# PlatonB/ld-tools

Measured on AMD Instinct MI355X. Metric: SNP-pairs/sec (r2+D'), higher is better.
Workload: dtype fp4 (E2M1 0/1 operands, exact f32 accumulation)

## Files before the change

### ld_tools_amd/csrc/ldx_mfma.hip

```cpp
#include <stdlib.h>
#include <string.h>

#include <atomic>
#include <type_traits>

#include "ldx_common.h"
#include "ldx_tile.h"

namespace ldx {

typedef int v4i __attribute__((ext_vector_type(4)));
typedef int v16i __attribute__((ext_vector_type(16)));
typedef unsigned v4u __attribute__((ext_vector_type(4)));
typedef unsigned v2u __attribute__((ext_vector_type(2)));
typedef float v4f __attribute__((ext_vector_type(4)));
typedef int v8i __attribute__((ext_vector_type(8)));
typedef float v16f __attribute__((ext_vector_type(16)));

__device__ __forceinline__ void gload16_s(v4u &dst, uint32_t voff, const void *sbase)
{
    const void *t;
    asm volatile("s_mov_b64 %1, %3\n\tglobal_load_dwordx4 %0, %2, %1" : "=v"(dst), "=&s"(t) : "v"(voff), "s"(sbase));
}
__device__ __forceinline__ void gload16x2_s(v4u &dst0, v4u &dst1, uint32_t voff, const void *sbase)
// ... 290 lines not shown
                const uint32_t x = (my_xcd + k) & 7u;
                const uint32_t lo = aa.pass_base[(uint32_t)((uint64_t)n_slabs * x / 8u)], hi = aa.pass_base[(uint32_t)((uint64_t)n_slabs * (x + 1u) / 8u)];
                if (lo == hi) continue;
                const uint32_t got = atomicAdd(&sched[2u + 32u * x], 1u);
                if (got < hi - lo) return aa.order ? aa.order[lo + got] : lo + got;
            }
            return 0xFFFFFFFFu;
        } else {
            if (!sched) return static_next += gridDim.x;
            return gridDim.x + atomicAdd(&sched[0], 1u);
        }
    };
    uint32_t *ktok = nullptr;
    if (!kArea && sched && (ablate_arg & 4096)) {
        const uint32_t hw = __builtin_amdgcn_s_getreg(63492), xcc = __builtin_amdgcn_s_getreg(63508);
        ktok = sched + 2u + ((((xcc & 7u) * 8u + ((hw >> 13) & 7u)) * 2u + ((hw >> 12) & 1u)) * 16u + ((hw >> 8) & 15u));
    }
    uint32_t parity = 0;
    if (tid == 0) tickets[0] = kArea ? draw() : blockIdx.x;

    uint64_t hit_slot = 0, hit_slot_end = 0;
    uint32_t t_prev = 0xFFFFFFFFu;
    for (;;) {
        block_sync();
        const uint32_t ticket = tickets[parity];
        parity ^= 1u;
        if (kArea ? ticket == 0xFFFFFFFFu : ticket >= n_tickets) {
            if (tid == 0 && sched && atomicAdd(&sched[1], 1u) == gridDim.x - 1u) {
                store_agent(&sched[1], 0u);
                if (kArea)
                    for (uint32_t x = 0; x < 8u; ++x) store_agent(&sched[2u + 32u * x], 0u);
                asm volatile("s_waitcnt vmcnt(0)" ::: "memory");
                store_agent(&sched[0], 0u);
            }
            break;
        }
        const bool short_pass = !kArea && ticket >= n_norm;
        const uint32_t hsel = short_pass ? (ticket - n_norm) & 1u : 0u;
        const uint32_t seq = short_pass ? n_norm + ((ticket - n_norm) >> 1) : ticket;
        uint32_t p = p_begin + seq;
        auto pbase = [&](uint32_t tile) { return kArea ? aa.pass_base[tile] : mfma_pass_base(tile, n_slabs); };
        auto tile_of_pass = [&](uint32_t pp) {
            uint32_t lo = 0, hi = n_slabs;
            while (hi - lo > 1) {
                const uint32_t mid = (lo + hi) / 2;
                if (pbase(mid) <= pp) lo = mid; else hi = mid;
            }
            return lo;
        };
        uint32_t t;
        if (kArea && (ticket & kAreaDecoded)) {
            t = (ticket >> 12) & 0xFFFu;
            p = pbase(t) + (ticket & 0xFFFu);
        } else
#ifndef LDX_AB_FORWARD_TILES
        if constexpr (!kArea) {
            const uint32_t mirrored = p_end - 1u - seq;
            t = tile_of_pass(mirrored);
            const uint32_t lo_t = pbase(t) > p_begin ? pbase(t) : p_begin;
            const uint32_t hi_t = (t + 1u < n_slabs && pbase(t + 1u) < p_end) ? pbase(t + 1u) : p_end;
            p = lo_t + (hi_t - 1u - mirrored);
        } else
#endif
        {
            t = tile_of_pass(p);
        }
        const bool new_tile = t != t_prev;
        t_prev = t;
        const uint64_t tb = base64(t), te = base64(t + 1u);
        const uint64_t area_first = kArea ? tb + (aa.g_begin[t] - 2u * t) : 0u;
        const uint64_t pass = (kArea ? area_first : tb) + (uint64_t)(p - pbase(t)) * kMfmaWaves;
        const uint64_t seg_begin = kArea ? area_first : (v_begin > tb ? v_begin : tb);
        const uint64_t seg_end = kArea ? tb + (aa.g_end[t] > 2u * t ? aa.g_end[t] - 2u * t : 0u) : (v_end < te ? v_end : te);
        const uint32_t b_off = kFp4 ? ((tid >> 7) * kSlab + (tid & 127u)) * 16u : (tid >> 1) * kBRow + (tid & 1u) * 64u;
        const uint32_t nblocks = kFp4 ? nchunks / 2u : nchunks;

        auto pass_body = [&](auto mm_c) {
            constexpr int MM = decltype(mm_c)::value;
            const uint64_t vv = pass + wave;
            const bool active = vv >= seg_begin && vv < seg_end;
            const uint32_t g64 = (uint32_t)((vv < te ? vv : pass) - tb) + 2u * t;
            const uint32_t roff = MM == 1 ? 32u * hsel : 0u;
            const uint32_t row0 = g64 * kRows64 + roff;
            const uint4 *ai = alt + ((size_t)(row0 / kSlab) * nchunks) * kSlab + (row0 % kSlab) + l32 + (kFp4 ? half * kSlab : 0u);
            constexpr uint32_t kAStride = kFp4 ? 2u * kSlab : kSlab;

            typedef std::conditional_t<kFp4, v16f, v16i> acc_t;
            typedef std::conditional_t<kFp4, float, int> accel_t;
            auto count_of = [](accel_t x) { if constexpr (kFp4) return (uint32_t)x; else return (uint32_t)x >> 3; };
            acc_t acc[MM][4];
#pragma unroll
            for (int m = 0; m < MM; ++m)
#pragma unroll
                for (int tt = 0; tt < 4; ++tt)
#pragma unroll
                    for (int e = 0; e < 16; ++e) acc[m][tt][e] = 0;

            auto read_bf = [&](v4i (&bf)[4], const unsigned char *buf, int w) {
#pragma unroll
                for (int tt = 0; tt < 4; ++tt)
#ifdef LDX_AB_NOBREAD
                    bf[tt] = v4i{(int)(uintptr_t)buf + w + tt, 1, 1, 1};
#else
                    bf[tt] = kFp4 ? *reinterpret_cast<const v4i *>(buf + (((uint32_t)w * 2u + half) * kSlab + 32u * tt + l32) * 16u)
                                  : *reinterpret_cast<const v4i *>(buf + (32u * tt + l32) * kBRow + w * 32u + half * 16u);
#endif
            };
            auto mma8 = [&](const v4i (&af)[MM], const v4i (&bf)[4]) {
#pragma unroll
                for (int m = 0; m < MM; ++m)
#pragma unroll
                    for (int tt = 0; tt < 4; ++tt)
#ifdef LDX_AB_NOMFMA
                        asm volatile("" : "+v"(acc[m][tt]) : "v"(af[m]), "v"(bf[tt]));
#else
                    {
                        if constexpr (kFp4) {
                            const v8i a8v = {af[m].x, af[m].y, af[m].z, af[m].w, 0, 0, 0, 0};
                            const v8i b8v = {bf[tt].x, bf[tt].y, bf[tt].z, bf[tt].w, 0, 0, 0, 0};
                            acc[m][tt] = __builtin_amdgcn_mfma_scale_f32_32x32x64_f8f6f4(a8v, b8v, acc[m][tt], 4, 4, 0, 0, 0, 0);
                        } else {
                            acc[m][tt] = __builtin_amdgcn_mfma_i32_32x32x32_i8(af[m], bf[tt], acc[m][tt], 0, 0, 0);
                        }
                    }
#endif
            };
            auto interleave = [&]() {
                __builtin_amdgcn_sched_group_barrier(0x100, 4, 0);
#pragma unroll
                for (int k = 0; k < 4 * MM; ++k) {
                    __builtin_amdgcn_sched_group_barrier(0x008, 1, 0);
                    __builtin_amdgcn_sched_group_barrier(0x002, LDX_VALU_PER_MFMA, 0);
                }
            };
            auto lds_barrier = [&]() {
                __builtin_amdgcn_sched_barrier(0);
#ifndef LDX_AB_NOBARRIER
                __builtin_amdgcn_s_waitcnt(0xC07F);
                __builtin_amdgcn_s_barrier();
#endif
                __builtin_amdgcn_sched_barrier(0);
            };

            LDX_STAMP(0);
            v4u ar[3][MM];
            auto touch_ring = [&](int k) {
                if constexpr (MM == 2) asm volatile("" : "+v"(ar[k][0]), "+v"(ar[k][1]));
                else asm volatile("" : "+v"(ar[k][0]));
            };
            typedef std::conditional_t<kFp4, v4u, v2u> bring_t;
            bring_t br[3];
            auto clampc = [&](uint32_t c) { return c < nblocks ? c : nblocks - 1u; };
            constexpr uint32_t kBlockBytes = kAStride * 16u;
            const uint32_t b_voff = kFp4 ? (uint32_t)((((size_t)t * nchunks + (tid >> 7)) * kSlab + (tid & 127u)) * 16u)
                                         : (uint32_t)(((size_t)t * nchunks * kSlab) * 16u + tid * 8u);
            const uint32_t a_voff = (uint32_t)((size_t)(ai - alt) * 16u);
            auto block_base = [&](uint32_t blk) { return reinterpret_cast<const unsigned char *>(alt) + (size_t)blk * kBlockBytes; };
            auto load_b = [&](bring_t &dst, uint32_t blk) {
                if constexpr (kFp4) gload16_s(dst, b_voff, block_base(blk));
                else gload8_s(dst, b_voff, block_base(blk));
            };
            auto load_a = [&](v4u (&dst)[MM], uint32_t blk) {
                if constexpr (MM == 2) gload16x2_s(dst[0], dst[1], a_voff, block_base(blk));
                else gload16_s(dst[0], a_voff, block_base(blk));
            };
            auto bquarter = [&](unsigned char *buf, const bring_t &bits, int q) {
// ... 97 lines not shown
            block_sync();
            LDX_STAMP(1);
            if (ablate & 32) __builtin_amdgcn_s_setprio(2);
#if defined(LDX_AB_BANDPRIO)
            if (kArea) { if (LDX_AB_BANDPRIO == 1 ? (blockIdx.x >= gridDim.x / 2u) : (blockIdx.x & 1u)) __builtin_amdgcn_s_setprio(1); else __builtin_amdgcn_s_setprio(0); }
#endif
            v4i af0[MM], bf0[4], af1[MM], bf1[4];
            read_bf(bf0, bexp, 0);
#pragma unroll
            for (int m = 0; m < MM; ++m) af0[m] = expand_a(ar[0][m].x);

            const uint32_t nch_run = (ablate & 2) ? 1u : nblocks;
#ifdef LDX_CHUNK_STAMPS
            unsigned long long cst[6] = {0, 0, 0, 0, 0, 0};
#endif
#define LDX_CHUNK(CUR, NXT, FAR, cc)                                                                               \
            {                                                                                                      \
                const uint32_t c_ = (cc);                                                                          \
                const unsigned char *rd = bexp + (c_ & 1u) * kBBuf;                                                \
                unsigned char *wr = bexp + ((c_ + 1u) & 1u) * kBBuf;                                               \
                const uint32_t c3 = clampc(c_ + 2u);                                                               \
                LDX_CSTAMP(0)                                                                                      \
                 \
                       \
                load_b(br[FAR], c3);                                                                               \
                load_a(ar[FAR], c3);                                                                               \
                asm volatile("s_waitcnt vmcnt(%0)" : : "n"(MM == 2 ? 5 : 3));    \
                asm volatile("" : "+v"(br[NXT]));                                                                  \
                      \
                read_bf(bf1, rd, 1);                                                                               \
                _Pragma("unroll") for (int m = 0; m < MM; ++m) af1[m] = expand_a(ar[CUR][m].y);               \
                bquarter(wr, br[NXT], 1);                                                                          \
                mma8(af0, bf0);                                                                                    \
                interleave();                                                                                      \
                __builtin_amdgcn_sched_barrier(0);                                                                 \
                LDX_CSTAMP(1)                                                                                      \
                                             \
                read_bf(bf0, rd, 2);                                                                               \
                _Pragma("unroll") for (int m = 0; m < MM; ++m) af0[m] = expand_a(ar[CUR][m].z);               \
                bquarter(wr, br[NXT], 2);                                                                          \
                mma8(af1, bf1);                                                                                    \
                interleave();                                                                                      \
                __builtin_amdgcn_sched_barrier(0);                                                                 \
                LDX_CSTAMP(2)                                                                                      \
                                             \
                read_bf(bf1, rd, 3);                                                                               \
                _Pragma("unroll") for (int m = 0; m < MM; ++m) af1[m] = expand_a(ar[CUR][m].w);               \
                bquarter(wr, br[NXT], 3);                                                                          \
                mma8(af0, bf0);                                                                                    \
                interleave();                                                                                      \
                __builtin_amdgcn_sched_barrier(0);                                                                 \
                LDX_CSTAMP(3)                                                                                      \
                lds_barrier();                        \
                LDX_CSTAMP(4)                                                                                      \
                   \
                 \
                           \
                asm volatile("s_waitcnt vmcnt(%0)" : : "n"(MM));                                                   \
                touch_ring(NXT);                                                                                   \
                asm volatile("" : "+v"(br[FAR]));                                                                  \
                read_bf(bf0, wr, 0);                                                                               \
                _Pragma("unroll") for (int m = 0; m < MM; ++m) af0[m] = expand_a(ar[NXT][m].x);               \
                bquarter(bexp + (c_ & 1u) * kBBuf, br[FAR], 0);                                                    \
                mma8(af1, bf1);                                                                                    \
                interleave();                                                                                      \
                __builtin_amdgcn_sched_barrier(0);                                                                 \
                LDX_CSTAMP(5)                                                                                      \
            }
#define LDX_CHUNK_IDLE(NXT, FAR, cc)                                                                               \
            {                                                                                                      \
                const uint32_t c_ = (cc);                                                                          \
                unsigned char *wr = bexp + ((c_ + 1u) & 1u) * kBBuf;                                               \
                load_b(br[FAR], clampc(c_ + 2u));                                                                  \
                asm volatile("s_waitcnt vmcnt(1)");                                 \
                asm volatile("" : "+v"(br[NXT]));                                                                  \
                bquarter(wr, br[NXT], 1);                                                                          \
                bquarter(wr, br[NXT], 2);                                                                          \
                bquarter(wr, br[NXT], 3);                                                                          \
                lds_barrier();                                                                                     \
                asm volatile("s_waitcnt vmcnt(0)");                                                                \
                asm volatile("" : "+v"(br[FAR]));                                                                  \
                bquarter(bexp + (c_ & 1u) * kBBuf, br[FAR], 0);                                                    \
            }
            if (__builtin_expect(!active, 0)) {
                for (uint32_t c = 0; c < nch_run; c += 3) {
                    LDX_CHUNK_IDLE(1, 2, c)
                    if (c + 1 < nch_run) LDX_CHUNK_IDLE(2, 0, c + 1)
                    if (c + 2 < nch_run) LDX_CHUNK_IDLE(0, 1, c + 2)
                }
            } else {
#ifdef LDX_AB_PEEL
            if constexpr (!kArea) {
                LDX_CHUNK(0, 1, 2, 0u)
                for (uint32_t c = 1; c < nch_run; c += 3) {
                    LDX_CHUNK(1, 2, 0, c)
                    if (c + 1 < nch_run) LDX_CHUNK(2, 0, 1, c + 1)
                    if (c + 2 < nch_run) LDX_CHUNK(0, 1, 2, c + 2)
                }
            } else
#endif
            {
                for (uint32_t c = 0; c < nch_run; c += 3) {
                    LDX_CHUNK(0, 1, 2, c)
                    if (c + 1 < nch_run) LDX_CHUNK(1, 2, 0, c + 1)
                    if (c + 2 < nch_run) LDX_CHUNK(2, 0, 1, c + 2)
                }
            }
            }
#undef LDX_CHUNK
#undef LDX_CHUNK_IDLE
            asm volatile("s_waitcnt vmcnt(0)");
            touch_ring(0);
            touch_ring(1);
            touch_ring(2);
            asm volatile("" : "+v"(br[0]), "+v"(br[1]), "+v"(br[2]));

#ifdef LDX_CHUNK_STAMPS
            asm volatile("s_waitcnt lgkmcnt(0)");
            if (my_stamps && lane == 0 && npass == 1)
                for (int k = 0; k < 6; ++k) my_stamps[6 + 4 * (kStampPasses - 2) + k] = cst[k];
#endif
            LDX_STAMP(2);
            uint32_t next_ticket = 0;
            if (tid == 0) {
                if (ktok) atomicExch(ktok, 0u);
                next_ticket = draw();
            }
            if (ablate & 32) __builtin_amdgcn_s_setprio(0);
            else if (!(ablate & 16)) __builtin_amdgcn_s_setprio(3);
            if constexpr (kScore) {
                block_sync();
            } else if (!active) {
                if (tid == 0) tickets[parity] = next_ticket;
                return;
            }
            typedef double d2 __attribute__((ext_vector_type(2)));
            double fa2[4], fr2[4];
            double sfa = 0.0, sfr = 0.0, sq = 0.0;
#pragma unroll
            for (int tt = 0; tt < 4; ++tt) {
                if (kRaw) {
                    fa2[tt] = fa[t * kSlab + 32u * tt + l32];
                    fr2[tt] = fr[t * kSlab + 32u * tt + l32];
                }
            }
            if (kRaw) {
                const uint32_t il = row0 + (MM == 1 ? l32 : lane);
                sfa = fa[il];
                sfr = fr[il];
                sq = q[il];
            }
            auto epilogue = [&](auto clean_c) {
#pragma unroll 1
            for (int e = 0; e < 16; ++e) {
                constexpr bool kClean = decltype(clean_c)::value;
                uint32_t ri[MM], cnt[MM][4];
                uint64_t us[MM];
                bool in_range[MM], valid[MM][4], slow[MM][4];
                Cell res[MM][4];
                ldx_ld64 rw[MM][4];
                bool any_slow = false;
#pragma unroll
                for (int m = 0; m < MM; ++m) {
                    ri[m] = 32u * m + (e & 3) + 8u * (e >> 2) + 4u * half;
                    us[m] = vv * 8u + (ri[m] + roff) / kGroup;
                    in_range[m] = kClean || (us[m] >= u_begin && us[m] < u_end);
                }
// ... 15 lines not shown
                } else {
                    FastRow fr2x[MM];
#pragma unroll
                    for (int m = 0; m < MM; ++m) {
                        const d2 *rs = reinterpret_cast<const d2 *>(rstat + ri[m] * kStat);
                        const d2 r01 = rs[0], r23 = rs[1];
                        fr2x[m] = FastRow{r01.x, r01.y, r23.x, r23.y};
                    }
                    constexpr int kPairs = MM == 2 ? 4 : 2;
                    auto chain_m = [](int, int k) { return MM == 2 ? k : 0; };
                    auto chain_tt = [](int pp, int k) { return MM == 2 ? pp : 2 * pp + k; };
                    auto load_col = [&](int tt) {
                        const d2 *cs = reinterpret_cast<const d2 *>(cstat + (32u * tt + l32) * kStat);
                        const d2 c01 = cs[0], c23 = cs[1];
                        return FastCol{c01.x, c01.y, c23.x, c23.y};
                    };
                    FastCol nxt[2];
                    nxt[0] = load_col(chain_tt(0, 0));
                    nxt[1] = MM == 2 ? nxt[0] : load_col(chain_tt(0, 1));
#pragma unroll
                    for (int pp = 0; pp < kPairs; ++pp) {
                        const FastCol fcx[2] = {nxt[0], nxt[1]};
                        if (pp + 1 < kPairs) {
                            nxt[0] = load_col(chain_tt(pp + 1, 0));
                            nxt[1] = MM == 2 ? nxt[0] : load_col(chain_tt(pp + 1, 1));
                        }
                        FastRow frk[2];
                        accel_t a8[2];
                        Cell r2[2];
                        bool s2[2];
#pragma unroll
                        for (int k = 0; k < 2; ++k) {
                            const int m = chain_m(pp, k), tt = chain_tt(pp, k);
                            frk[k] = fr2x[m];
                            const uint32_t i = row0 + ri[m], j = t * kSlab + 32u * tt + l32;
                            valid[m][tt] = kClean || ((i > j) && (i < n_snps));
                            a8[k] = acc[m][tt][e];
                        }
                        if (ablate & 1) {
#pragma unroll
                            for (int k = 0; k < 2; ++k) {
                                res[chain_m(pp, k)][chain_tt(pp, k)] = encode_cell<Cell>((double)a8[k], 0.0, false, false);
                                slow[chain_m(pp, k)][chain_tt(pp, k)] = false;
                            }
                        } else {
                            ld_multi_fast2<2, kClean, Cell>(a8, fk, frk, fcx, r2, s2);
#pragma unroll
                            for (int k = 0; k < 2; ++k) {
                                const int m = chain_m(pp, k), tt = chain_tt(pp, k);
                                res[m][tt] = r2[k];
                                slow[m][tt] = s2[k] && valid[m][tt];
                                any_slow = any_slow || slow[m][tt];
                            }
                        }
                    }
                    if (__builtin_expect(__any(any_slow), 0)) {
#pragma unroll
                        for (int m = 0; m < MM; ++m)
#pragma unroll
                            for (int tt = 0; tt < 4; ++tt)
                                if (slow[m][tt]) {
                                    const uint32_t i = row0 + ri[m], j = t * kSlab + 32u * tt + l32;
                                    res[m][tt] = encode_cell<Cell>(
                                        ld_pair_mirror((double)count_of(acc[m][tt][e]) / n, fa[i], fr[i], q[i], fa[j], fr[j]));
                                }
                    }
                }
#pragma unroll
                for (int m = 0; m < MM; ++m)
                    if (in_range[m] && !(ablate & 4)) {
#pragma unroll
                        for (int tt = 0; tt < 4; ++tt) {
                            const uint32_t jl = 32u * tt + l32;
                            const size_t o = (size_t)(us[m] - u_begin) * LDX_UNIT_PAIRS + cell_offset<Cell>((ri[m] + roff) % kGroup, jl);
                            Cell w = res[m][tt];
                            if (!kClean && !valid[m][tt]) w = zero_cell<Cell>();
                            store_cell(out + o, w);
                            if (kRaw) raw[o] = rw[m][tt];
                            if (kN11) n11[o] = valid[m][tt] ? count_of(acc[m][tt][e]) : 0u;
                        }
                    }
            }
            };
            auto epilogue_f32 = [&](bool all_ordinary) -> bool {
              if constexpr (kF32Tier) {
                if (ablate & 1) return true;
                const uint64_t ub = vv * 8u - u_begin;
                Cell *const ubase = out + (((uint64_t)__builtin_amdgcn_readfirstlane((uint32_t)(ub >> 32)) << 32) |
                                           __builtin_amdgcn_readfirstlane((uint32_t)ub)) * LDX_UNIT_PAIRS;
                uint32_t ln = lane;
                asm volatile("" : "+v"(ln));
                const uint32_t l32e = ln & 31u, halfe = ln >> 5;
                const uint32_t lane_off = halfe * 4u * kSlab + (sizeof(Cell) <= 4 ? 4u : 2u) * l32e;
                const uint32_t lane_off_b = lane_off * (uint32_t)sizeof(Cell);
                const float *const rt = rtab32 + halfe * 16u, *const ct = ctab32 + l32e * 4u;
                const uint32_t grp0 = roff / kGroup;
                uint32_t qn = 0;
                F32Col cols[4];
#pragma unroll
                for (int tt = 0; tt < 4; ++tt) {
                    const v4f v = *reinterpret_cast<const v4f *>(ct + 32u * tt * 4u);
                    cols[tt] = F32Col{v.x, v.y, v.z, v.w};
                }
                uint64_t colmask[4], rdeg;
#pragma unroll
                for (int tt = 0; tt < 4; ++tt) colmask[tt] = __builtin_amdgcn_ballot_w64(f32_entry_degenerate(cols[tt].ra, cols[tt].s));
                {
                    const v4f rv = *reinterpret_cast<const v4f *>(rtab32 + (MM == 1 ? l32e : ln) * 4u);
                    rdeg = __builtin_amdgcn_ballot_w64(f32_entry_degenerate(rv.y, rv.w));
                }
#ifdef LDX_AB_NODEGSEL
                const bool any_deg = false;
#else
                const bool any_deg = (rdeg | colmask[0] | colmask[1] | colmask[2] | colmask[3]) != 0ull;
#endif
                float cal[4] = {0.0f, 0.0f, 0.0f, 0.0f};
                if (!f32_small_n((double)fc32.n)) {
#pragma unroll
                    for (int tt = 0; tt < 4; ++tt) f32_split_a(cols[tt].a, cols[tt].a, cal[tt]);
                }
                auto steps = [&](auto small_c, auto deg_c) -> bool {
                constexpr bool kDeg = decltype(deg_c)::value;
                [[maybe_unused]] const uint32_t forced = sizeof(Cell) == 4 ? ((uint32_t)LDX_K16_INT0 << 16 | LDX_K16_INT0) : 0x80000000u;
                auto load_rows = [&](int e, F32Row (&dst)[MM]) {
#pragma unroll
                    for (int m = 0; m < MM; ++m) {
                        const v4f v = *reinterpret_cast<const v4f *>(rt + (32u * m + (e & 3) + 8u * (e >> 2)) * 4u);
                        dst[m] = F32Row{v.x, v.y, v.z, v.w};
                    }
                };
#ifdef LDX_ROW_PREFETCH
                static_assert(LDX_STEP_UNROLL % 2 == 0, "LDX_ROW_PREFETCH alternates two row buffers: unroll by an even number");
                F32Row rowbuf[2][MM];
                load_rows(0, rowbuf[0]);
#endif
#pragma unroll 1
                for (int e_ = 0; e_ < 16; e_ += LDX_STEP_UNROLL) {
#pragma unroll
                for (int r_ = 0; r_ < LDX_STEP_UNROLL; ++r_) {
                    const int e = e_ + r_;
#if defined(LDX_TUNING) && defined(LDX_STAMPS_ONLY)
                    if (my_stamps && lane == 0 && npass == 1) my_stamps[6 + 4 * kStampPasses + e] = __builtin_amdgcn_s_memtime();
#endif
#ifdef LDX_ROW_PREFETCH
                    F32Row (&rows)[MM] = rowbuf[r_ & 1];
                    load_rows((e + 1) & 15, rowbuf[(r_ + 1) & 1]);
#else
                    F32Row rows[MM];
                    load_rows(e, rows);
#endif
                    constexpr int kOne = cell_measure<Cell>::value;
                    Cell cell[4 * MM];
                    uint32_t cellw[2 * MM];
                    float wmax = 0.0f, ymin = 1.0f;
#pragma unroll
                    for (int g = 0; g < MM; ++g) {
                        float c4[4];
                        F32Row r4[4];
#pragma unroll
                        for (int tt = 0; tt < 4; ++tt) {
                            c4[tt] = acc[g][tt][e];
                            r4[tt] = rows[g];
                        }
                        uint64_t rowmask = 0;
                        if constexpr (kDeg) {
                            const uint32_t ri0 = 32u * g + (e & 3) + 8u * (e >> 2);
                            rowmask = (((rdeg >> ri0) & 1ull) ? 0x00000000FFFFFFFFull : 0ull) |
                                      (((rdeg >> (ri0 + 4u)) & 1ull) ? 0xFFFFFFFF00000000ull : 0ull);
                        }
                        if constexpr (kOne >= 0) {
                            uint32_t b4[4];
                            ld_multi_f32_one<4, kOne, decltype(small_c)::value, !decltype(small_c)::value>(c4, fc32, r4, cols, b4, wmax, ymin, cal);
                            if constexpr (kDeg) {
#pragma unroll
                                for (int tt = 0; tt < 4; ++tt) b4[tt] = select_lanes(b4[tt], (uint32_t)LDX_K16_INT0, rowmask | colmask[tt]);
                            }
                            cellw[2 * g] = __builtin_amdgcn_perm(b4[1], b4[0], 0x05040100u);
                            cellw[2 * g + 1] = __builtin_amdgcn_perm(b4[3], b4[2], 0x05040100u);
                        } else {
                            Cell o4[4];
                            ld_multi_f32<4, Cell, decltype(small_c)::value, !decltype(small_c)::value>(c4, fc32, r4, cols, o4, wmax, ymin, cal);
                            if constexpr (kDeg) {
#pragma unroll
                                for (int tt = 0; tt < 4; ++tt) {
                                    const uint64_t m = rowmask | colmask[tt];
                                    if constexpr (sizeof(Cell) == 4) {
                                        o4[tt] = __builtin_bit_cast(Cell, select_lanes(__builtin_bit_cast(uint32_t, o4[tt]), forced, m));
                                    } else {
                                        const v2u w = __builtin_bit_cast(v2u, o4[tt]);
                                        o4[tt] = __builtin_bit_cast(Cell, v2u{select_lanes(w.x, forced, m), select_lanes(w.y, forced, m)});
                                    }
                                }
                            }
#pragma unroll
                            for (int tt = 0; tt < 4; ++tt) cell[g * 4 + tt] = o4[tt];
                        }
                    }
                    const bool sure = ((wmax < fc32.tol) & (ymin > 0.0f)) | ((ablate & 1024) != 0);
#ifdef LDX_AB_NOSTORE
                    if (sure) {
                        uint32_t x = 0;
#pragma unroll
                        for (int q8 = 0; q8 < 4 * MM; ++q8) { if constexpr (sizeof(Cell) == 2) x ^= cellw[q8 / 2]; else if constexpr (sizeof(Cell) == 4) x ^= __builtin_bit_cast(uint32_t, cell[q8]); else x ^= (uint32_t)__builtin_bit_cast(unsigned long long, cell[q8]) ^ (uint32_t)(__builtin_bit_cast(unsigned long long, cell[q8]) >> 32); }
                        asm volatile("" : : "v"(x));
                    }
                    if (false) {
#else
                    if (sure && !(ablate & 4)) {
#endif
#pragma unroll
                        for (int m = 0; m < MM; ++m) {
                            Cell *const row = ubase + ((4u * m + grp0 + (e >> 2)) * LDX_UNIT_PAIRS + (e & 3) * kSlab);
                            if constexpr (kOne >= 0) store_words2_saddr(row, lane_off_b, cellw[2 * m], cellw[2 * m + 1]);
                            else store_cells4_saddr(row, lane_off_b, cell[m * 4 + 0], cell[m * 4 + 1], cell[m * 4 + 2], cell[m * 4 + 3]);
                        }
                    }
#ifdef LDX_AB_OLD_BALLOT
                    const unsigned long long parked = __ballot(!sure);
#else
                    const unsigned long long parked = __builtin_amdgcn_ballot_w64(!sure);
#endif
                    if (parked) {
                        const uint32_t np = (uint32_t)__builtin_popcountll(parked);
                        if (qn + np > kQueueCap) {
                            LDX_COUNT(2, 1);
                            return false;
                        }
                        if (!sure) {
                            const uint32_t pos = qn + __builtin_amdgcn_mbcnt_hi((uint32_t)(parked >> 32),
                                                                              __builtin_amdgcn_mbcnt_lo((uint32_t)parked, 0u));
                            qid[pos] = ((uint32_t)e << 8) | ln;
                            v4f *dst = reinterpret_cast<v4f *>(qcnt + (size_t)pos * 8u);
#pragma unroll
                            for (int m = 0; m < MM; ++m) dst[m] = v4f{acc[m][0][e], acc[m][1][e], acc[m][2][e], acc[m][3][e]};
                        }
                        qn += np;
                    }
                }
                }
#if defined(LDX_TUNING) && defined(LDX_STAMPS_ONLY)
                    if (my_stamps && lane == 0 && npass == 1) my_stamps[6 + 4 * kStampPasses + 16] = __builtin_amdgcn_s_memtime();
#endif
                    return true;
                };
                const bool small_n = f32_small_n((double)fc32.n);
                const bool done = any_deg ? (small_n ? steps(std::true_type{}, std::true_type{}) : steps(std::false_type{}, std::true_type{}))
                                          : (small_n ? steps(std::true_type{}, std::false_type{}) : steps(std::false_type{}, std::false_type{}));
                if (!done) return false;
                LDX_COUNT(0, 1);
                LDX_COUNT(1, qn);
                if ((ablate & 2048) != 0) qn = 0;
                if (qn) {
                    __builtin_amdgcn_s_waitcnt(0xC07F);
                    __builtin_amdgcn_wave_barrier();
                }
                uint32_t ld = ln;
                asm volatile("" : "+v"(ld));
                constexpr uint32_t kPer = 4u * MM, kShift = MM == 2 ? 3u : 2u;
                auto pair_of = [&](uint32_t ent, uint32_t pr, uint32_t &ri2, uint32_t &cl) {
                    const uint32_t id = qid[ent];
                    const uint32_t e2 = id >> 8, l2 = id & 31u, h2 = (id >> 5) & 1u;
                    ri2 = 32u * (pr >> 2) + (e2 & 3u) + 8u * (e2 >> 2) + 4u * h2;
                    cl = 32u * (pr & 3u) + l2;
                    return qcnt[(size_t)ent * 8u + pr];
                };
                auto mirror_cell = [&](float cnt, uint32_t ri2, uint32_t cl) {
                    const uint32_t i = row0 + ri2, j = t * kSlab + cl;
#if defined(LDX_TUNING) && !defined(LDX_STAMPS_ONLY)
                    atomicAdd(&g_dbg[3], 1ull);
#endif
                    return encode_cell<Cell>(ld_pair_mirror((double)cnt / n, fa[i], fr[i], q[i], fa[j], fr[j]));
                };
                auto cell_at = [&](uint32_t ri2, uint32_t cl) -> Cell & {
                    return ubase[(size_t)(grp0 + ri2 / kGroup) * LDX_UNIT_PAIRS + cell_offset<Cell>(ri2 % kGroup, cl)];
                };
                uint32_t un = 0;
                for (uint32_t q0 = 0; q0 < qn; q0 += 64u / kPer) {
                    const uint32_t ent = q0 + (ld >> kShift), pr = ld & (kPer - 1u);
                    const bool live = ent < qn;
                    uint32_t ri2 = 0, cl = 0;
                    Cell r2[1] = {zero_cell<Cell>()};
                    bool s2[1] = {false};
                    float a2[1] = {0.0f};
                    if (live) {
                        a2[0] = pair_of(ent, pr, ri2, cl);
                        const d2 *rs = reinterpret_cast<const d2 *>(rstat + ri2 * kStat);
                        const d2 r01 = rs[0], r23 = rs[1];
                        const FastRow frk[1] = {FastRow{r01.x, r01.y, r23.x, r23.y}};
                        const d2 *cs = reinterpret_cast<const d2 *>(cstat + cl * kStat);
                        const d2 c01 = cs[0], c23 = cs[1];
                        const FastCol fcx[1] = {FastCol{c01.x, c01.y, c23.x, c23.y}};
                        if (all_ordinary) ld_multi_fast2<1, true, Cell>(a2, fk, frk, fcx, r2, s2);
                        else ld_multi_fast2<1, false, Cell>(a2, fk, frk, fcx, r2, s2);
                    }
                    const bool unsure = live && s2[0];
                    const unsigned long long um = __ballot(unsure);
                    bool deferred = false;
                    if (um) {
                        const uint32_t pos = un + __builtin_amdgcn_mbcnt_hi((uint32_t)(um >> 32), __builtin_amdgcn_mbcnt_lo((uint32_t)um, 0u));
                        deferred = unsure && pos < 64u;
                        if (deferred) ulist[pos] = (ent << 3) | pr;
                        un += (uint32_t)__builtin_popcountll(um);
                        if (__builtin_expect(un > 64u, 0)) {
                            if (unsure && !deferred) r2[0] = mirror_cell(a2[0], ri2, cl);
                        }
                    }
                    if (live && !deferred) cell_at(ri2, cl) = r2[0];
                }
                if (un) {
                    __builtin_amdgcn_s_waitcnt(0xC07F);
                    __builtin_amdgcn_wave_barrier();
                    if (ld < (un < 64u ? un : 64u)) {
                        const uint32_t id = ulist[ld];
                        uint32_t ri2, cl;
                        const float cnt = pair_of(id >> 3, id & 7u, ri2, cl);
                        cell_at(ri2, cl) = mirror_cell(cnt, ri2, cl);
                    }
                }
                return true;
              } else {
                return false;
              }
            };
            auto epilogue_r32 = [&]() {
              if constexpr (kR32) {
                const uint64_t ub = vv * 8u - u_begin;
                const uint64_t ubs = ((uint64_t)__builtin_amdgcn_readfirstlane((uint32_t)(ub >> 32)) << 32) |
                                     __builtin_amdgcn_readfirstlane((uint32_t)ub);
                uint32_t ln = lane;
                asm volatile("" : "+v"(ln));
                const uint32_t l32e = ln & 31u, halfe = ln >> 5;
                const uint32_t lane_off_b = (halfe * 4u * kSlab + 4u * l32e) * (uint32_t)sizeof(Cell);
                const uint32_t grp0 = roff / kGroup;
                double ca[4], cs[4];
#pragma unroll
                for (int tt = 0; tt < 4; ++tt) {
                    const d2s c = *reinterpret_cast<const d2s *>(cstat + (32u * tt + l32e) * kStat);
                    ca[tt] = c.x;
                    cs[tt] = c.y;
                }
                const uint32_t j0 = t * kSlab + l32e;
                const bool all_valid = row0 >= (t + 1u) * kSlab && row0 + 32u * MM <= n_snps;
#pragma unroll 1
                for (int e = 0; e < 16; ++e) {
#pragma unroll
                    for (int m = 0; m < MM; ++m) {
                        const uint32_t g = 4u * m + grp0 + (uint32_t)(e >> 2);
                        const uint64_t us = vv * 8u + g;
                        if (us < u_begin || us >= u_end) continue;
                        accel_t c4[4];
#pragma unroll
                        for (int tt = 0; tt < 4; ++tt) {
                            c4[tt] = acc[m][tt][e];
                            asm volatile("" : "+v"(c4[tt]));
                        }
                        const uint32_t ri = 32u * m + (uint32_t)(e & 3) + 8u * (uint32_t)(e >> 2) + 4u * halfe;
                        const d2s rw = *reinterpret_cast<const d2s *>(rstat + ri * kStat);
                        const uint32_t i = row0 + ri;
                        Cell o4[4];
#pragma unroll
                        for (int tt = 0; tt < 4; ++tt) {
                            const double cnt = kFp4 ? (double)c4[tt] : (double)((uint32_t)c4[tt] >> 3);
                            o4[tt] = r32_cell(cnt, n, rw.x, rw.y, ca[tt], cs[tt]);
                            if (!all_valid && !(i > j0 + 32u * tt && i < n_snps)) o4[tt] = zero_cell<Cell>();
                        }
                        Cell *const row = out + ((ubs + g) * LDX_UNIT_PAIRS + (uint32_t)(e & 3) * kSlab);
                        store_cells4_saddr(row, lane_off_b, o4[0], o4[1], o4[2], o4[3]);
                    }
                }
              }
            };
            uint64_t *const score_cols = reinterpret_cast<uint64_t *>(bexp);
            auto score_epilogue = [&](uint32_t st) {
              if constexpr (kScore) {
                const double win = aa.flank;
                uint64_t *const rows_lds = reinterpret_cast<uint64_t *>(ctab32) + wave * (kRows64 * 9u);
// ... 220 lines not shown
                        rqs[m] = r23.y;
                    }
#pragma unroll
                    for (int tt = 0; tt < 4; ++tt) {
                        if (!((tt_live >> tt) & 1u)) continue;
                        const d2 *cs = reinterpret_cast<const d2 *>(cstat + (32u * tt + l32) * kStat);
                        const d2 c01 = cs[0], c23 = cs[1];
                        const uint32_t j = t * kSlab + 32u * tt + l32;
                        bool cand[2];
                        accel_t a8[2];
#pragma unroll
                        for (int m = 0; m < 2; ++m) {
                            a8[m] = acc[m][tt][e];
                            asm volatile("" : "+v"(a8[m]));
                        }
#pragma unroll
                        for (int m = 0; m < 2; ++m) {
                            const uint32_t i = row0 + ri[m];
                            cand[m] = (i > j) && (i < n_snps);
                            if (prefilter) {
                                const double dn4 = __builtin_fma((double)a8[m], fk.nsc, -(ras[m] * c01.x));
                                double y;
                                if (aa.measure == LDX_MEASURE_RSQ) {
                                    y = (dn4 * (rqs[m] * c23.y)) * dn4;
                                } else {
                                    const bool neg = dn4 < 0.0;
                                    const double x = neg ? c01.y : c23.x, yy = neg ? c23.x : c01.y;
                                    y = __builtin_fabs(dn4) * max_raw(rra[m] * x, rrr[m] * yy);
                                }
                                cand[m] = cand[m] && (y >= kcand);
                            }
                        }
                        if (!__any(cand[0] || cand[1])) continue;
                        if (aqn + 128u > kAreaQueue) drain();
#pragma unroll
                        for (int m = 0; m < 2; ++m) {
                            const unsigned long long mask = __ballot(cand[m]);
                            if (cand[m]) {
                                const uint32_t pos = aqn + __builtin_amdgcn_mbcnt_hi((uint32_t)(mask >> 32), __builtin_amdgcn_mbcnt_lo((uint32_t)mask, 0u));
                                aq_id[pos] = ((uint32_t)e << 9) | ((uint32_t)m << 8) | ((uint32_t)tt << 6) | lane;
                                aq_cnt[pos] = __builtin_bit_cast(uint32_t, a8[m]);
                            }
                            aqn += (uint32_t)__builtin_popcountll(mask);
                        }
                    }
                }
                drain();
                hit_slot = slot;
                hit_slot_end = slot_end;
              }
            };
            if constexpr (kScore) {
                const uint32_t st = 1u + (uint32_t)aa.measure;
                if (active) score_epilogue(st);
                block_sync();
                uint64_t *const sums = reinterpret_cast<uint64_t *>(aa.hits);
                for (uint32_t f = tid; f < kSlab * st; f += kMfmaThreads) {
                    uint64_t v = 0;
#pragma unroll
                    for (uint32_t w = 0; w < (uint32_t)kMfmaWaves; ++w)
                        if (pass + w >= seg_begin && pass + w < seg_end) v += score_cols[w * (kSlab * 9u) + f];
                    const uint32_t j = t * kSlab + f / st;
                    if (v != 0u && j < n_snps) atomicAdd(reinterpret_cast<unsigned long long *>(sums) + (size_t)j * st + f % st, (unsigned long long)v);
                }
                if (tid == 0) tickets[parity] = next_ticket;
                if (!(ablate & 16)) __builtin_amdgcn_s_setprio(0);
                return;
            }
            if constexpr (kArea) {
                area_epilogue();
                if (tid == 0) tickets[parity] = next_ticket;
                if (!(ablate & 16)) __builtin_amdgcn_s_setprio(0);
#ifdef LDX_TUNING
                LDX_STAMP(3);
                ++npass;
                if (my_stamps && lane == 0) {
                    my_stamps[3] = npass;
                    my_stamps[4] = __builtin_amdgcn_s_memrealtime();
                    my_stamps[5] = __builtin_amdgcn_s_memtime();
                }
#endif
                return;
            }
            const bool inside = !kRaw && row0 >= (t + 1u) * kSlab && row0 + 32u * MM <= n_snps && (t + 1u) * kSlab <= n_snps &&
                                vv * 8u >= u_begin && vv * 8u + 8u <= u_end;
            const bool all_ordinary = rows_ordinary && (cols_odd[0] | cols_odd[1]) == 0u;
            const bool clean = inside && all_ordinary;
            if constexpr (kR32) {
                epilogue_r32();
            } else if constexpr (kF32Tier) {
                if (inside && !(ablate & 512) && epilogue_f32(all_ordinary)) {
                } else if (clean && !(ablate & 512)) {
                    epilogue(std::true_type{});
                } else {
                    epilogue(std::false_type{});
                }
            } else {
                if (clean && !(ablate & 512)) epilogue(std::true_type{});
                else epilogue(std::false_type{});
            }
            if (tid == 0) tickets[parity] = next_ticket;
            if (!(ablate & 16)) __builtin_amdgcn_s_setprio(0);
#ifdef LDX_TUNING
            LDX_STAMP(3);
            ++npass;
            if (my_stamps && lane == 0) {
                my_stamps[3] = npass;
                my_stamps[4] = __builtin_amdgcn_s_memrealtime();
                my_stamps[5] = __builtin_amdgcn_s_memtime();
            }
#endif
        };
        if constexpr (kArea) {
            pass_body(std::integral_constant<int, 2>{});
        } else {
#ifdef LDX_MM1
            pass_body(std::integral_constant<int, 1>{});
#else
            if (short_pass) pass_body(std::integral_constant<int, 1>{});
            else pass_body(std::integral_constant<int, 2>{});
#endif
        }
    }
    if (kArea)
        for (uint64_t sl = hit_slot + lane; sl < hit_slot_end; sl += 64u)
            if (sl < aa.hit_cap) aa.hits[sl].query = 0xFFFFFFFFu;
}

template <bool kRaw, bool kN11, bool kFp4, typename Cell>
static int launch_mfma(const void *alt, const double *fa, const double *fr, const double *q, uint32_t n_snps,
                       uint32_t n_hap, uint64_t unit_begin, uint64_t unit_end, Cell *out, ldx_ld64 *out_raw,
                       uint32_t *out_n11, uint32_t *sched, hipStream_t s)
{
    const uint32_t nch = n_chunks(n_hap);
    if ((uint64_t)n_slabs(n_snps) * nch * kSlab * 16u >= (1ull << 32)) {
        set_error("ld_triangle on the matrix pipe: a bit plane of 4 GiB or more (%u SNPs x %u haplotypes)", n_snps, n_hap);
        return kNoMatrixPath;
    }
    const size_t lds = mfma_lds_bytes(kStatRows, kFp4 && !kRaw && !kN11 && !std::is_same<Cell, ldx_r32>::value);
    if (lds > 64u * 1024u) {
        static std::atomic<uint64_t> opted{0};
        int dev = 0;
        LDX_HIP(hipGetDevice(&dev));
        if (dev < 0 || dev >= 64 || !((opted.load(std::memory_order_relaxed) >> dev) & 1u)) {
            LDX_HIP(hipFuncSetAttribute((const void *)triangle_mfma_kernel<kRaw, kN11, false, kFp4, Cell>,
                                        hipFuncAttributeMaxDynamicSharedMemorySize, (int)lds));
            if (dev >= 0 && dev < 64) opted.fetch_or(1ull << dev, std::memory_order_relaxed);
        }
    }
    const int cus = device_cus();
    const uint32_t ns = n_slabs(n_snps);
    const uint64_t G64 = (uint64_t)ns * 2u;
    auto base64 = [&](uint64_t t) { return t * G64 - t * (t - 1u); };
    auto tile_of = [&](uint64_t v) {
        uint32_t lo = 0, hi = ns;
        while (hi - lo > 1) {
            const uint32_t mid = (lo + hi) / 2;
            if (base64(mid) <= v) lo = mid; else hi = mid;
        }
        return lo;
    };
    const uint64_t v_begin = unit_begin / 8u, v_end = (unit_end + 7u) / 8u;
    const uint32_t t0 = tile_of(v_begin), t1 = tile_of(v_end - 1u);
    const uint32_t p_begin = mfma_pass_base(t0, ns) + (uint32_t)((v_begin - base64(t0)) / kMfmaWaves);
    const uint32_t p_end = mfma_pass_base(t1, ns) + (uint32_t)((v_end - base64(t1) + kMfmaWaves - 1u) / kMfmaWaves);
    const uint64_t slots = (uint64_t)cus * kWgPerCu;
    const uint32_t n_pass = p_end - p_begin;
    uint32_t n_short = 2ull * n_pass <= slots ? n_pass : (n_pass > slots ? (uint32_t)(slots / 4u) : 0u);
    const int forced = g_forced_short.load(std::memory_order_relaxed);
    if (forced >= 0) n_short = (uint32_t)forced < n_pass ? (uint32_t)forced : n_pass;
#ifdef LDX_MM1
    n_short = n_pass;
#endif
    uint64_t grid = slots;
// ... 476 lines not shown
```

Before: 421.6 billion.

## Route edge tiles through f32 epilogue with masking and skip MFMA for pad-only rows

Passes whose rows lie entirely beyond n_snps are now treated as idle for the MFMA loop and write zeros directly in the f32 epilogue. Edge (non-interior) tiles that cover whole units now use the fast f32 epilogue too, with per-lane masks that zero cells outside the lower triangle or past n_snps, instead of falling back to the slower generic epilogue. The aim is to cut work on diagonal and boundary tiles. In exchange, it adds mask computation on the degenerate path and needs the masking to be correct at the triangle boundary.

```diff
diff --git a/ld_tools_amd/csrc/ldx_mfma.hip b/ld_tools_amd/csrc/ldx_mfma.hip
--- a/ld_tools_amd/csrc/ldx_mfma.hip
+++ b/ld_tools_amd/csrc/ldx_mfma.hip
@@ -396,6 +396,8 @@
             const uint32_t g64 = (uint32_t)((vv < te ? vv : pass) - tb) + 2u * t;
             const uint32_t roff = MM == 1 ? 32u * hsel : 0u;
             const uint32_t row0 = g64 * kRows64 + roff;
+            const bool pad_only = kF32Tier && row0 >= n_snps;
+            const bool counting = active && !pad_only;
             const uint4 *ai = alt + ((size_t)(row0 / kSlab) * nchunks) * kSlab + (row0 % kSlab) + l32 + (kFp4 ? half * kSlab : 0u);
             constexpr uint32_t kAStride = kFp4 ? 2u * kSlab : kSlab;
 
@@ -659,7 +661,7 @@
                 asm volatile("" : "+v"(br[FAR]));                                                                  \
                 bquarter(bexp + (c_ & 1u) * kBBuf, br[FAR], 0);                                                    \
             }
-            if (__builtin_expect(!active, 0)) {
+            if (__builtin_expect(!counting, 0)) {
                 for (uint32_t c = 0; c < nch_run; c += 3) {
                     LDX_CHUNK_IDLE(1, 2, c)
                     if (c + 1 < nch_run) LDX_CHUNK_IDLE(2, 0, c + 1)
@@ -841,7 +843,7 @@
                     }
             }
             };
-            auto epilogue_f32 = [&](bool all_ordinary) -> bool {
+            auto epilogue_f32 = [&](bool all_ordinary, bool edge) -> bool {
               if constexpr (kF32Tier) {
                 if (ablate & 1) return true;
                 const uint64_t ub = vv * 8u - u_begin;
@@ -854,6 +856,12 @@
                 const uint32_t lane_off_b = lane_off * (uint32_t)sizeof(Cell);
                 const float *const rt = rtab32 + halfe * 16u, *const ct = ctab32 + l32e * 4u;
                 const uint32_t grp0 = roff / kGroup;
+                if (pad_only) {
+#pragma unroll 1
+                    for (uint32_t k = 0; k < 4u * MM * (uint32_t)sizeof(Cell); ++k)
+                        store_cells4_saddr(reinterpret_cast<uint32_t *>(ubase + grp0 * LDX_UNIT_PAIRS) + k * 256u, ln * 16u, 0u, 0u, 0u, 0u);
+                    return true;
+                }
                 uint32_t qn = 0;
                 F32Col cols[4];
 #pragma unroll
@@ -881,6 +889,14 @@
                 auto steps = [&](auto small_c, auto deg_c) -> bool {
                 constexpr bool kDeg = decltype(deg_c)::value;
                 [[maybe_unused]] const uint32_t forced = sizeof(Cell) == 4 ? ((uint32_t)LDX_K16_INT0 << 16 | LDX_K16_INT0) : 0x80000000u;
+                [[maybe_unused]] auto outside = [&](uint32_t i0, int tt) -> uint64_t {
+                    const uint32_t j0 = t * kSlab + 32u * (uint32_t)tt;
+                    auto half32 = [&](uint32_t i) -> uint32_t {
+                        const uint32_t lim = i < n_snps ? i : 0u;
+                        return lim <= j0 ? 0xFFFFFFFFu : (lim - j0 >= 32u ? 0u : 0xFFFFFFFFu << (lim - j0));
+                    };
+                    return (uint64_t)half32(i0) | ((uint64_t)half32(i0 + 4u) << 32);
+                };
                 auto load_rows = [&](int e, F32Row (&dst)[MM]) {
 #pragma unroll
                     for (int m = 0; m < MM; ++m) {
@@ -933,6 +949,10 @@
                             if constexpr (kDeg) {
 #pragma unroll
                                 for (int tt = 0; tt < 4; ++tt) b4[tt] = select_lanes(b4[tt], (uint32_t)LDX_K16_INT0, rowmask | colmask[tt]);
+                                if (edge) {
+#pragma unroll
+                                    for (int tt = 0; tt < 4; ++tt) b4[tt] = select_lanes(b4[tt], 0u, outside(row0 + 32u * g + (e & 3) + 8u * (e >> 2), tt));
+                                }
                             }
                             cellw[2 * g] = __builtin_amdgcn_perm(b4[1], b4[0], 0x05040100u);
                             cellw[2 * g + 1] = __builtin_amdgcn_perm(b4[3], b4[2], 0x05040100u);
@@ -950,6 +970,18 @@
                                         o4[tt] = __builtin_bit_cast(Cell, v2u{select_lanes(w.x, forced, m), select_lanes(w.y, forced, m)});
                                     }
                                 }
+                                if (edge) {
+#pragma unroll
+                                    for (int tt = 0; tt < 4; ++tt) {
+                                        const uint64_t m = outside(row0 + 32u * g + (e & 3) + 8u * (e >> 2), tt);
+                                        if constexpr (sizeof(Cell) == 4) {
+                                            o4[tt] = __builtin_bit_cast(Cell, select_lanes(__builtin_bit_cast(uint32_t, o4[tt]), 0u, m));
+                                        } else {
+                                            const v2u w = __builtin_bit_cast(v2u, o4[tt]);
+                                            o4[tt] = __builtin_bit_cast(Cell, v2u{select_lanes(w.x, 0u, m), select_lanes(w.y, 0u, m)});
+                                        }
+                                    }
+                                }
                             }
 #pragma unroll
                             for (int tt = 0; tt < 4; ++tt) cell[g * 4 + tt] = o4[tt];
@@ -1003,7 +1035,7 @@
                     return true;
                 };
                 const bool small_n = f32_small_n((double)fc32.n);
-                const bool done = any_deg ? (small_n ? steps(std::true_type{}, std::true_type{}) : steps(std::false_type{}, std::true_type{}))
+                const bool done = (any_deg || edge) ? (small_n ? steps(std::true_type{}, std::true_type{}) : steps(std::false_type{}, std::true_type{}))
                                           : (small_n ? steps(std::true_type{}, std::false_type{}) : steps(std::false_type{}, std::false_type{}));
                 if (!done) return false;
                 LDX_COUNT(0, 1);
@@ -1051,6 +1083,13 @@
                         const FastCol fcx[1] = {FastCol{c01.x, c01.y, c23.x, c23.y}};
                         if (all_ordinary) ld_multi_fast2<1, true, Cell>(a2, fk, frk, fcx, r2, s2);
                         else ld_multi_fast2<1, false, Cell>(a2, fk, frk, fcx, r2, s2);
+                        if (edge) {
+                            const uint32_t i = row0 + ri2, j = t * kSlab + cl;
+                            if (!(i > j && i < n_snps)) {
+                                r2[0] = zero_cell<Cell>();
+                                s2[0] = false;
+                            }
+                        }
                     }
                     const bool unsure = live && s2[0];
                     const unsigned long long um = __ballot(unsure);
@@ -1437,14 +1476,15 @@
 #endif
                 return;
             }
-            const bool inside = !kRaw && row0 >= (t + 1u) * kSlab && row0 + 32u * MM <= n_snps && (t + 1u) * kSlab <= n_snps &&
-                                vv * 8u >= u_begin && vv * 8u + 8u <= u_end;
+            const bool interior = row0 >= (t + 1u) * kSlab && row0 + 32u * MM <= n_snps && (t + 1u) * kSlab <= n_snps;
+            const bool whole = vv * 8u >= u_begin && vv * 8u + 8u <= u_end;
+            const bool inside = !kRaw && interior && whole;
             const bool all_ordinary = rows_ordinary && (cols_odd[0] | cols_odd[1]) == 0u;
             const bool clean = inside && all_ordinary;
             if constexpr (kR32) {
                 epilogue_r32();
             } else if constexpr (kF32Tier) {
-                if (inside && !(ablate & 512) && epilogue_f32(all_ordinary)) {
+                if (whole && !(ablate & 512) && epilogue_f32(all_ordinary, !interior)) {
                 } else if (clean && !(ablate & 512)) {
                     epilogue(std::true_type{});
                 } else {
```

New measurement: 439.6 billion (median of 6 runs). 1.04x the previous value.
